# sloisel/MultiGridBarrier.jl

Measured on AMD Instinct MI355X. Metric: Newton iters/sec + wall-clock to converge, 2D P2 p-Laplace L=9, higher is better.
Workload: dtype f64

## Files before the change

### multigridbarrier.jl_amd/csrc/mf_launch_plan.hpp

```cpp
#pragma once
#include <algorithm>
#include <cstdint>
#include <cstdlib>
#include <vector>

#include "mf_analysis.hpp"

namespace mgbhip {

struct MfLaunch {
    int32_t first, count;
    int32_t cls;
    int32_t max_m, max_k;
    int32_t max_child = 0;
    bool tiny = false;
    bool wave = false;
    bool inv = false;
    bool iface = false;
    int32_t grec_first = -1;
};

constexpr int BIG_INV_MAX_M = 7000;
constexpr int GATHER_MAX_CHILD = 8;
constexpr int BIG_DIAG0_MIN_COUNT = 24;

struct MfSwitches {
    bool no_geo;
    bool old_big;
    bool merge_groups;
    bool packed_leaves;
    bool wave_small;
    int64_t inv_min_n;
    int64_t wave_min_n;
    bool gather_lds_maps;
    int gather_ct;
    static MfSwitches from_env() {
        auto on = [](const char* name) { const char* e = getenv(name); return e && e[0] == '1'; };
        auto num = [](const char* name, long long dflt) { const char* e = getenv(name); return e ? atoll(e) : dflt; };
        return {on("MGBHIP_NO_GEO"), on("MGBHIP_OLD_BIG"), !on("MGBHIP_NO_MERGE_GROUPS"), !on("MGBHIP_NO_PACKED_LEAVES"),
                !on("MGBHIP_NO_WAVE_SMALL"), num("MGBHIP_INV_MIN_N", 1024), num("MGBHIP_WAVE_MIN_N", 0),
                on("MGBHIP_GATHER_LDS_MAPS"), (int)num("MGBHIP_GATHER_CT", 0)};
    }
};

using LevelLaunches = std::vector<std::vector<MfLaunch>>;

inline MfLaunch launch_of_range(const MfPlan& plan, MfLaunch L, int32_t first, int32_t count) {
    L.first = first; L.count = count;
    L.max_m = 0; L.max_k = 0; L.max_child = 0;
    for (int32_t t = first; t < first + count; ++t) {
        L.max_m = std::max(L.max_m, plan.fronts[t].m);
        L.max_k = std::max(L.max_k, plan.fronts[t].k);
        L.max_child = std::max(L.max_child, plan.fronts[t].nchild);
    }
    return L;
}

inline void merge_straggler_groups(const MfPlan& plan, std::vector<MfLaunch>& G) {
    auto absorb = [&](size_t into, size_t from) {
        MfLaunch& A = G[into];
        const MfLaunch& B = G[from];
        A.first = B.first;
        A.count += B.count;
        A.max_k = std::max(A.max_k, B.max_k);
        A.max_child = std::max(A.max_child, B.max_child);
        G.erase(G.begin() + (long)from);
    };
    if (G.size() >= 2 && G.back().cls == 0 && G.back().inv) {
        int64_t lds_count = 0;
        bool ok = true;
        for (size_t g = 0; g + 1 < G.size(); ++g) { lds_count += G[g].count; ok = ok && !G[g].tiny && plan.fronts[G[g].first].m > 32; }
        if (ok && lds_count <= G.back().count)
            while (G.size() >= 2) absorb(G.size() - 1, G.size() - 2);
    }
    for (size_t g = 0; g + 1 < G.size();) {
        const bool next_lds = G[g + 1].cls != 0;
        if (next_lds && !G[g].tiny && (G[g].count < 256 || 4 * (int64_t)G[g].count < G[g + 1].count)) absorb(g + 1, g);
        else ++g;
    }
}

inline void split_interface_front(const MfPlan& plan, LevelLaunches& levels, bool inv_allowed) {
    const int32_t q = plan.iface_front;
    for (auto& G : levels) {
        for (size_t g = 0; g < G.size(); ++g) {
            const MfLaunch L = G[g];
            if (q < L.first || q >= L.first + L.count) continue;
            std::vector<MfLaunch> out;
            if (q > L.first) out.push_back(launch_of_range(plan, L, L.first, q - L.first));
            MfLaunch I = launch_of_range(plan, L, q, 1);
            I.cls = 0; I.tiny = false; I.wave = false; I.iface = true;
            I.inv = (I.max_m <= BIG_INV_MAX_M && inv_allowed);
            out.push_back(I);
            if (q + 1 < L.first + L.count) out.push_back(launch_of_range(plan, L, q + 1, L.first + L.count - q - 1));
// ... 57 lines not shown
        MfLaunch S{};
        for (auto& L : levels[l]) {
            if (!L.cls || L.tiny) { solves[l].push_back(L); continue; }
            if (S.count == 0) S = L;
            else {
                S.count += L.count;
                S.max_m = std::max(S.max_m, L.max_m);
                S.max_k = std::max(S.max_k, L.max_k);
            }
        }
        if (S.count) solves[l].insert(solves[l].begin(), S);
    }
    return solves;
}

inline std::vector<char> fronts_on_big_path(const MfPlan& plan, const LevelLaunches& levels) {
    std::vector<char> on_big_path(plan.fronts.size(), 0);
    for (auto& lev : levels)
        for (auto& L : lev)
            if (!L.cls)
                for (int32_t q = L.first; q < L.first + L.count; ++q) on_big_path[q] = 1;
    return on_big_path;
}

inline bool leaf_fronts_packable(const MfPlan& plan, const LevelLaunches& levels, const std::vector<char>& on_big_path) {
    bool any = false;
    for (auto& lev : levels)
        for (auto& L : lev)
            if (L.tiny)
                for (int32_t q = L.first; q < L.first + L.count; ++q) {
                    const int32_t par = plan.fronts[q].parent;
                    if (par >= 0 && on_big_path[par]) return false;
                    any = true;
                }
    return any;
}

enum MfAssembly : int32_t { MF_ASM_NONE = 0, MF_ASM_GATHER = 1, MF_ASM_COLS = 2 };
enum MfBlock0 : int32_t { MF_B0_NA = 0, MF_B0_GATHER = 1, MF_B0_DIAG0 = 2, MF_B0_STEP0 = 3 };
enum MfBackward : int32_t { MF_BWD_NA = 0, MF_BWD_K8 = 1, MF_BWD_K16 = 2, MF_BWD_GENERAL = 3 };

inline size_t big_gather_lds(const MfLaunch& L) { return (size_t)L.max_child * (size_t)L.max_m * sizeof(int32_t); }
inline MfAssembly big_assembly_kind(const MfLaunch& L) {
    if (L.cls) return MF_ASM_NONE;
    if (L.max_child < 1 || L.max_child > GATHER_MAX_CHILD || big_gather_lds(L) > 40 * 1024) return MF_ASM_COLS;
    return MF_ASM_GATHER;
}
inline MfBlock0 big_block0_kind(const MfLaunch& L, bool inv) {
    if (L.cls || !inv) return MF_B0_NA;
    if (!L.iface && big_assembly_kind(L) == MF_ASM_GATHER) return MF_B0_GATHER;
    return (L.iface || L.count >= BIG_DIAG0_MIN_COUNT) ? MF_B0_DIAG0 : MF_B0_STEP0;
}
inline int backward_small_kmax(const MfLaunch& L) { return L.max_k <= 8 ? 8 : (L.max_k <= 16 ? 16 : 0); }

constexpr int GATHER_MIN_WGS = 768;
inline int big_gather_ct(const MfLaunch& L, int forced) {
    if (forced == 8 || forced == 16 || forced == 32) return forced;
    int ct = 8;
    while (ct < 32 && (int64_t)L.count * ((L.max_m + 2 * ct - 1) / (2 * ct)) >= GATHER_MIN_WGS) ct *= 2;
    return ct;
}

struct GatherRec {
    int64_t map_off;
    int64_t base[GATHER_MAX_CHILD];
    int32_t ld[GATHER_MAX_CHILD];
    int32_t bs[GATHER_MAX_CHILD];
};

inline void build_gather_maps(const MfPlan& plan, LevelLaunches& levels, std::vector<GatherRec>& recs, std::vector<int32_t>& gmap) {
    recs.clear();
    gmap.clear();
    for (auto& lev : levels)
        for (auto& L : lev) {
            L.grec_first = -1;
            if (L.count == 0 || big_assembly_kind(L) != MF_ASM_GATHER) continue;
            L.grec_first = (int32_t)recs.size();
            for (int32_t q = L.first; q < L.first + L.count; ++q) {
                const Front& f = plan.fronts[q];
                GatherRec R{};
                R.map_off = (int64_t)gmap.size();
                gmap.resize(gmap.size() + (size_t)f.nchild * (size_t)f.m, -1);
                for (int32_t c = 0; c < f.nchild; ++c) {
                    const Front& ch = plan.fronts[plan.children[f.child_off + c]];
                    R.base[c] = ch.F_off + (int64_t)ch.k * ch.m + ch.k;
                    R.ld[c] = ch.m;
                    R.bs[c] = ch.m - ch.k;
                    int32_t* mp = gmap.data() + R.map_off + (int64_t)c * f.m;
                    for (int32_t j = 0; j < ch.m - ch.k; ++j) mp[plan.rel[ch.rel_off + j]] = j;
                }
                recs.push_back(R);
            }
        }
}

constexpr int MF_LAUNCH_ROW = 16;
inline int64_t launch_rows(const LevelLaunches& levels, const LevelLaunches& solves, bool leaf_packed, bool robust,
                           int32_t* out, int64_t cap) {
    int64_t n = 0;
    for (size_t l = 0; l < levels.size(); ++l) {
        int32_t bwd = 0;
        for (auto& S : solves[l])
            if (S.cls && !S.tiny) { const int km = backward_small_kmax(S); bwd = km == 8 ? MF_BWD_K8 : (km == 16 ? MF_BWD_K16 : MF_BWD_GENERAL); }
        for (auto& L : levels[l]) {
            if (n < cap && out) {
                const bool inv = L.inv && !robust;
                int32_t* r = out + n * MF_LAUNCH_ROW;
                r[0] = (int32_t)l; r[1] = L.first; r[2] = L.count; r[3] = L.cls; r[4] = L.max_m; r[5] = L.max_k; r[6] = L.max_child;
                r[7] = L.tiny; r[8] = L.wave; r[9] = inv; r[10] = L.iface; r[11] = L.tiny && leaf_packed;
                r[12] = big_assembly_kind(L); r[13] = big_block0_kind(L, inv); r[14] = (L.cls && !L.tiny) ? bwd : (int32_t)MF_BWD_NA; r[15] = 0;
            }
            ++n;
        }
    }
    return n;
}

}
```

### multigridbarrier.jl_amd/csrc/mf_numeric.hip

```cpp
#include <hip/hip_runtime.h>

#include <cstdio>

#include <algorithm>
#include <cstdlib>

#include "../../include/mgbhip.h"
#include "mf_solver.hpp"
#include "mf_device.hpp"
#include "mf_small.hpp"
#include "mf_big_subst.hpp"
#include "mf_big_inv.hpp"

namespace mgbhip {

namespace {

int32_t query_lds_cap() {
    if (hipFuncSetAttribute((const void*)mf_factor_small<8, true>, hipFuncAttributeMaxDynamicSharedMemorySize,
                            (int)factor_small_lds(128)) == hipSuccess)
        return 128;
    (void)hipGetLastError();
    return 88;
}
bool query_inv_optin() {
    if (hipFuncSetAttribute((const void*)mf_fwd_inv, hipFuncAttributeMaxDynamicSharedMemorySize, (int)fwd_inv_lds(BIG_INV_MAX_M)) == hipSuccess &&
        hipFuncSetAttribute((const void*)mf_bwd_inv, hipFuncAttributeMaxDynamicSharedMemorySize,
                            (int)bwd_inv_lds(BIG_INV_MAX_M, BIG_INV_MAX_M)) == hipSuccess)
        return true;
    (void)hipGetLastError();
    return false;
}

void build_gather_lists(const MfPlan& plan, const std::vector<char>& on_big_path, std::vector<FrontDev>& fd,
                        std::vector<int64_t>& ug_ptr, std::vector<int64_t>& ug_src) {
    for (int32_t i = 0; i < (int32_t)plan.fronts.size(); ++i) {
        const Front& f = plan.fronts[i];
        if (!on_big_path[i]) continue;
        fd[i].ug_off = (int64_t)ug_ptr.size();
        std::vector<int32_t> cnt((size_t)f.m + 1, 0);
        for (int32_t c = 0; c < f.nchild; ++c) {
            const Front& ch = plan.fronts[plan.children[f.child_off + c]];
            for (int32_t j = 0; j < ch.m - ch.k; ++j) cnt[plan.rel[ch.rel_off + j] + 1]++;
        }
        const int64_t base = (int64_t)ug_src.size();
        std::vector<int64_t> pos((size_t)f.m + 1);
        pos[0] = base;
        for (int32_t j = 0; j < f.m; ++j) pos[j + 1] = pos[j] + cnt[j + 1];
        ug_ptr.insert(ug_ptr.end(), pos.begin(), pos.end());
        ug_src.resize((size_t)pos[f.m]);
        std::vector<int64_t> fill(pos.begin(), pos.end() - 1);
        for (int32_t c = 0; c < f.nchild; ++c) {
            const Front& ch = plan.fronts[plan.children[f.child_off + c]];
            for (int32_t j = 0; j < ch.m - ch.k; ++j) ug_src[(size_t)fill[plan.rel[ch.rel_off + j]]++] = ch.u_off + j;
        }
    }
    if (ug_ptr.empty()) ug_ptr.push_back(0);
    if (ug_src.empty()) ug_src.push_back(0);
}

bool pack_leaf_fronts(const MfPlan& plan, const LevelLaunches& levels, const std::vector<char>& on_big_path,
                      std::vector<FrontDev>& fd) {
    if (!leaf_fronts_packable(plan, levels, on_big_path)) return false;
    for (auto& lev : levels)
        for (auto& L : lev)
            if (L.tiny)
                for (int32_t q = L.first; q < L.first + L.count; ++q) fd[q].packed = 1;
    return true;
}

std::vector<int32_t> remap_a_dst(const MfPlan& plan, const LevelLaunches& levels) {
    std::vector<int32_t> ad(plan.a_dst);
// ... 60 lines not shown
        const double one = 1.0;
        d_one.upload(&one, 1, st);
        MGB_HIP_CHECK(hipStreamSynchronize(st));
    }
    d_tbig.alloc(plan.front_idx.size() ? plan.front_idx.size() : 1);
    d_tsol.alloc(plan.front_idx.size() ? plan.front_idx.size() : 1);
    d_dvec.alloc(plan.front_idx.size() ? plan.front_idx.size() : 1);
    d_status.alloc(2);
    d_status.zero(st);
}

void MfSolver::analyze(int64_t n, const int32_t* rowptr, const int32_t* colidx, hipStream_t st,
                       const double* coords, int dim, bool protect_peeled, const int32_t* top, int64_t ntop) {
    const MfSwitches sw = MfSwitches::from_env();
    MfOptions opt;
    opt.protect_peeled = protect_peeled;
    opt.top = top;
    opt.ntop = ntop;
    opt.border = true;
    mf_analyze(n, rowptr, colidx, opt, plan, sw.no_geo ? nullptr : coords, dim);
    const int32_t nf = (int32_t)plan.fronts.size();
    std::vector<FrontDev> fd(nf);
    for (int32_t i = 0; i < nf; ++i) {
        const Front& f = plan.fronts[i];
        fd[i] = FrontDev{f.k, f.m, f.nchild, f.a_cnt, f.F_off, f.idx_off, f.u_off, f.child_off, f.rel_off, f.a_off, f.acol_off, -1, 0, 0};
    }
    upload_plan(st);

    lds_cap = query_lds_cap();
    const bool inv_ok = !sw.old_big && query_inv_optin();
    level_launches = classify_launches(plan, lds_cap, inv_ok, sw);
    level_solves = merge_level_solves(level_launches);
    uses_inv = false;
    const std::vector<char> on_big_path = fronts_on_big_path(plan, level_launches);
    int32_t max_big = 1;
    for (auto& lev : level_launches)
        for (auto& L : lev) {
            uses_inv = uses_inv || L.inv;
            if (!L.cls) max_big = std::max(max_big, L.count);
        }
    d_dscr.alloc((size_t)max_big * 2 * NB * NB);

    std::vector<int64_t> ug_ptr, ug_src;
    build_gather_lists(plan, on_big_path, fd, ug_ptr, ug_src);
    leaf_packed = sw.packed_leaves && pack_leaf_fronts(plan, level_launches, on_big_path, fd);
    d_ug_ptr.upload(ug_ptr, st);
    d_ug_src.upload(ug_src, st);
    std::vector<GatherRec> grec;
    std::vector<int32_t> gmap;
    if (!sw.gather_lds_maps) build_gather_maps(plan, level_launches, grec, gmap);
    gather_ct = sw.gather_ct;
    if (grec.empty()) { d_grec.release(); d_gmap.release(); }
    else { d_grec.upload(grec, st); d_gmap.upload(gmap, st); }
    d_fronts.upload(fd, st);
    h_fronts = fd;
    h_a_dst = remap_a_dst(plan, level_launches);
    d_a_dst.upload(h_a_dst, st);
    if (const char* e = getenv("MGBHIP_DEBUG"); e && atoi(e) >= 2) dump_plan(plan, level_launches);
    analyzed = true;
    MGB_HIP_CHECK(hipStreamSynchronize(st));
}

void MfSolver::set_direct_map(const int32_t* value_map, int64_t nnz, int64_t tail_base, hipStream_t st) {
    std::vector<int32_t> as(plan.a_src.size());
    for (size_t t = 0; t < as.size(); ++t) {
        const int64_t src = plan.a_src[t];
        const int64_t v = src < nnz ? (int64_t)value_map[src] : tail_base + (src - nnz);
        MGB_REQUIRE(v < (int64_t)INT32_MAX, "direct value index exceeds 32 bits");
        as[t] = (int32_t)v;
    }
    d_a_src_direct.upload(as, st);
    MGB_HIP_CHECK(hipStreamSynchronize(st));
}

void MfSolver::factor(const double* d_values, hipStream_t st, StageTimers* timers, bool direct, bool condensed) {
    MGB_REQUIRE(!direct || d_a_src_direct.n > 0, "MfSolver::factor: no direct value map");
    MGB_REQUIRE(!condensed || (direct && condensed_ok), "MfSolver::factor: condensed leaves are not enabled");
    MGB_REQUIRE(analyzed, "MfSolver::factor before analyze");
    const FactorArgs a{condensed ? d_fronts_c.p : d_fronts.p, d_children.p, d_rel.p,
                       condensed ? d_a_src_c.p : (direct ? d_a_src_direct.p : d_a_src.p), condensed ? d_a_dst_c.p : d_a_dst.p,
                       condensed ? d_a_colptr_c.p : d_a_colptr.p, d_values, d_arena.p, d_dscr.p, d_dvec.p, d_status.p, st,
                       d_grec.n ? d_grec.p : nullptr, d_gmap.p, gather_ct};
    if (timers) timers->begin("factor");
    factored_inv = !robust;
    if (!status_zero) MGB_HIP_CHECK(hipMemsetAsync(d_status.p, 0, sizeof(int32_t), st));
    status_zero = false;
    factored_condensed = condensed;
    int lvno = -1;
    for (auto& lev : level_launches) {
        LevelScope lvscope(timers, "fac", ++lvno);
        for (auto& L : lev) {
            if (L.count == 0) continue;
            if (condensed && lvno == 0) continue;
            if (L.tiny) launch_factor_tiny(a, L);
            else if (L.wave && L.cls <= 32) launch_factor_wave<32>(a, L);
            else if (L.wave) launch_factor_wave<48>(a, L);
            else if (L.cls) launch_factor_small(a, L);
            else {
                const bool inv = L.inv && !robust;
                const MfBlock0 b0 = big_block0_kind(L, inv);
                MGB_REQUIRE(!L.iface || (bool)iface_reduce, "MfSolver: interface front without a reduction hook");
                launch_big_assemble(a, L, b0 == MF_B0_GATHER);
                if (L.iface) {
                    const Front& fi = plan.fronts[L.first];
                    const int64_t tri = (int64_t)fi.m * (fi.m + 1) / 2;
                    d_ifpack.ensure((size_t)tri);
                    launch_tri_pack(fi.m, d_arena.p + fi.F_off, d_ifpack.p, false, st);
                    iface_reduce(d_ifpack.p, tri);
                    launch_tri_pack(fi.m, d_arena.p + fi.F_off, d_ifpack.p, true, st);
                }
                if (inv) {
                    if (b0 == MF_B0_DIAG0) launch_big_diag0(a, L, L.count);
                    launch_inv_steps(a, L, L.count, b0 == MF_B0_STEP0);
                } else
                    launch_subst_steps(a, L, L.count);
            }
        }
    }
    MGB_HIP_CHECK(hipGetLastError());
    if (timers) timers->end();
}

void MfSolver::solve(const double* d_b, double* d_x, hipStream_t st, StageTimers* timers) {
    MGB_REQUIRE(analyzed, "MfSolver::solve before analyze");
    if (timers) timers->begin("trisolve");
    const size_t n = (size_t)plan.n;
    MGB_HIP_CHECK(hipMemcpyAsync(d_bx.p, d_b, n * sizeof(double), hipMemcpyDeviceToDevice, st));
    MGB_HIP_CHECK(hipMemsetAsync(d_bx.p + n, 0, sizeof(double), st));
    forward_pass(d_bx.p, st, timers);
    backward_pass(d_xx.p, st, timers);
    MGB_HIP_CHECK(hipMemcpyAsync(d_x, d_xx.p, n * sizeof(double), hipMemcpyDeviceToDevice, st));
    MGB_HIP_CHECK(hipGetLastError());
    if (timers) timers->end();
}

// ... 175 lines not shown
```

### multigridbarrier.jl_amd/csrc/mf_small.hpp

```cpp
#pragma once
#include "mf_device.hpp"

namespace mgbhip {
namespace {

template <int NBT, bool PACKED>
__global__ void mf_factor_small(const FrontDev* __restrict__ fr, int32_t first,
                                const int32_t* __restrict__ children, const int32_t* __restrict__ rel,
                                const int32_t* __restrict__ a_src, const int32_t* __restrict__ a_dst,
                                const double* __restrict__ Hval, double* __restrict__ arena,
                                int32_t* __restrict__ status) {
    extern __shared__ double W[];
    const FrontDev F = fr[first + blockIdx.x];
    double* Fg = arena + F.F_off;
    const int m = F.m, k = F.k;
    const int tid = threadIdx.x, nt = blockDim.x;
    const int tx = tid % TX, ty = tid / TX, TYn = nt / TX;
    const int mm = PACKED ? m * (m + 1) / 2 : m * m;
    auto co = [m](int c) { return PACKED ? c * (m - 1) - c * (c - 1) / 2 : c * m; };
    double* S = W + mm;

    SP(0);
    int a_d0 = -1;
    double a_v0 = 0.0;
    if (tid < F.a_cnt) {
        a_d0 = a_dst[F.a_off + tid];
        a_v0 = Hval[a_src[F.a_off + tid]];
    }
    int64_t pU = 0, pR = 0;
    int32_t pM = 0, pB = 0;
    if (tid < min(CHILD_CHUNK, F.nchild)) {
        const FrontDev C = fr[children[F.child_off + tid]];
        child_update_desc(C, pU, pM);
        pR = C.rel_off;
        pB = C.m - C.k;
    }
    for (int i = tid; i < mm; i += nt) W[i] = 0.0;
    __syncthreads();
    if (a_d0 >= 0) W[a_d0] = a_v0;
    for (int t = tid + nt; t < F.a_cnt; t += nt) W[a_dst[F.a_off + t]] = Hval[a_src[F.a_off + t]];
    __syncthreads();
    SP(1);
    __shared__ int64_t cU[CHILD_CHUNK];
    __shared__ int64_t cR[CHILD_CHUNK];
    __shared__ int32_t cM[CHILD_CHUNK], cB[CHILD_CHUNK];
    __shared__ int32_t crl[128];
    __shared__ double prinv[32];
    for (int cbase = 0; cbase < F.nchild; cbase += CHILD_CHUNK) {
        const int nc = min(CHILD_CHUNK, F.nchild - cbase);
        __syncthreads();
        if (tid < nc) {
            if (cbase == 0) {
                cU[tid] = pU; cR[tid] = pR; cM[tid] = pM; cB[tid] = pB;
            } else {
                const FrontDev C = fr[children[F.child_off + cbase + tid]];
                int64_t u_; int32_t m_;
                child_update_desc(C, u_, m_);
                cU[tid] = u_;
                cR[tid] = C.rel_off;
                cM[tid] = m_;
                cB[tid] = C.m - C.k;
            }
        }
        __syncthreads();
        for (int c0 = 0; c0 < nc; c0 += 4) {
            if (nt == 256 && (c0 & 15) == 0) {
                const int ng = min(16, nc - c0);
                bool small16 = true;
                for (int u = 0; u < ng; ++u) small16 = small16 && cB[c0 + u] * cB[c0 + u] <= 64;
                if (small16) {
                    const int w = tid >> 6, e = tid & 63;
                    int dst[4];
                    double val[4];
#pragma unroll
                    for (int u = 0; u < 4; ++u) {
                        dst[u] = -1;
                        val[u] = 0.0;
                        const int c = c0 + 4 * w + u;
                        if (4 * w + u < ng) {
                            const int b = cB[c];
                            if (e < b * b) {
                                const int j = e / b, r = e - j * b;
                                if (r >= j) {
                                    const int32_t* rl = rel + cR[c];
                                    dst[u] = rl[r] + co(rl[j]);
                                    val[u] = arena[child_entry(cU[c], cM[c], j, r)];
                                }
                            }
                        }
                    }
#pragma unroll
                    for (int ph = 0; ph < 4; ++ph) {
                        if (4 * ph < ng) {
                            if (ph == w) {
#pragma unroll
                                for (int u = 0; u < 4; ++u) {
                                    if (dst[u] >= 0) W[dst[u]] += val[u];
                                    wave_sync();
                                }
                            }
                            __syncthreads();
                        }
                    }
                    c0 += 12;
                    continue;
                }
// ... 87 lines not shown
#pragma unroll
                for (int c = 0; c < NBT; ++c) {
                    S[c * m + r] = (c < nb) ? a[c] : 0.0;
                    if (c < nb) W[r + co(j0 + c)] = a[c] * prinv[c];
                }
            }
        }
        SPL(3);
        __syncthreads();
        SPL(4);
        {
            const int c0 = j0 + nb;
            const int T = (m - c0 + 15) >> 4;
            const int lane = tid & 63, fr16 = lane & 15, fk = lane >> 4;
            for (int tile = tid >> 6; tile < T * (T + 1) / 2; tile += nt >> 6) {
                int I = (int)((sqrtf(8.0f * (float)tile + 1.0f) - 1.0f) * 0.5f);
                while ((I + 1) * (I + 2) / 2 <= tile) ++I;
                while (I * (I + 1) / 2 > tile) --I;
                const int J = tile - I * (I + 1) / 2;
                const int r0 = c0 + 16 * I, cc0 = c0 + 16 * J;
                const int rr = min(r0 + fr16, m - 1), cc = min(cc0 + fr16, m - 1);
                double4_t acc = {0.0, 0.0, 0.0, 0.0};
#pragma unroll
                for (int kk = 0; kk < NBT / 4; ++kk) {
                    const int q = 4 * kk + fk;
                    const double sa = S[q * m + cc];
                    const double lb = (q < nb) ? W[rr + co(j0 + q)] : 0.0;
                    acc = __builtin_amdgcn_mfma_f64_16x16x4f64(sa, lb, acc, 0, 0, 0);
                }
#pragma unroll
                for (int i = 0; i < 4; ++i) {
                    const int col = cc0 + fk + 4 * i, row = r0 + fr16;
                    if (row < m && col < m && row >= col) W[row + co(col)] -= acc[i];
                }
            }
        }
        SPL(5);
        __syncthreads();
        SPL(6);
    }
    SP(3);
    if (bad && tid == 0) atomicOr(status, 1);
    if (PACKED) {
        for (int c = ty; c < m; c += TYn) {
            const int cc = co(c);
            for (int r = c + tx; r < m; r += TX) Fg[r + (int64_t)c * m] = W[cc + r];
        }
    } else {
        for (int i = tid; i < mm; i += nt) Fg[i] = W[i];
    }
    SP(4);
}

template <int MW>
__global__ __launch_bounds__(256) void mf_factor_wave(const FrontDev* __restrict__ fr, int32_t first, int32_t count,
                                                      const int32_t* __restrict__ children, const int32_t* __restrict__ rel,
                                                      const int32_t* __restrict__ a_src, const int32_t* __restrict__ a_dst,
                                                      const double* __restrict__ Hval, double* __restrict__ arena,
                                                      int32_t* __restrict__ status) {
    constexpr int PK = MW * (MW + 1) / 2;
    extern __shared__ double sh[];
#ifdef MGB_STEP_PROBE
#define WP(i) do { if (threadIdx.x == 0 && gridDim.x == 2048 && blockIdx.x == 1500) g_probe[8 + (i)] = wall_clock64(); } while (0)
#else
#define WP(i) do { } while (0)
#endif
    WP(0);
    const int lane = threadIdx.x & 63, wave = threadIdx.x >> 6;
    const int fi = blockIdx.x * 4 + wave;
    if (fi >= count) return;
    const FrontDev F = fr[first + fi];
    const int m = F.m, k = F.k;
    double* W = sh + (size_t)wave * PK;
    constexpr int WCH = 32;
    int64_t* cU = reinterpret_cast<int64_t*>(sh + (size_t)4 * PK) + wave * 2 * WCH;
    int64_t* cR = cU + WCH;
    int32_t* cM = reinterpret_cast<int32_t*>(reinterpret_cast<int64_t*>(sh + (size_t)4 * PK) + 4 * 2 * WCH) + wave * 2 * WCH;
    int32_t* cB = cM + WCH;
    auto pidx = [](int r, int c) { return c * MW - c * (c - 1) / 2 + (r - c); };
    int a_d0 = -1;
    double a_v0 = 0.0;
    if (lane < F.a_cnt) {
        a_d0 = a_dst[F.a_off + lane];
        a_v0 = Hval[a_src[F.a_off + lane]];
    }
    int64_t pU = 0, pR = 0;
    int32_t pM = 0, pB = 0;
    if (lane < min(WCH, F.nchild)) {
        const FrontDev C = fr[children[F.child_off + lane]];
        child_update_desc(C, pU, pM);
        pR = C.rel_off;
        pB = C.m - C.k;
    }
    for (int i = lane; i < PK; i += 64) W[i] = 0.0;
    wave_sync();
    WP(1);
    if (a_d0 >= 0) W[a_d0] = a_v0;
    for (int t = lane + 64; t < F.a_cnt; t += 64) W[a_dst[F.a_off + t]] = Hval[a_src[F.a_off + t]];
    wave_sync();
    WP(2);
    for (int cbase = 0; cbase < F.nchild; cbase += WCH) {
        const int nc = min(WCH, F.nchild - cbase);
        if (lane < nc) {
            if (cbase == 0) {
                cU[lane] = pU; cR[lane] = pR; cM[lane] = pM; cB[lane] = pB;
            } else {
                const FrontDev C = fr[children[F.child_off + cbase + lane]];
                int64_t u_; int32_t m_;
                child_update_desc(C, u_, m_);
                cU[lane] = u_;
                cR[lane] = C.rel_off;
                cM[lane] = m_;
                cB[lane] = C.m - C.k;
            }
        }
        wave_sync();
        for (int c0 = 0; c0 < nc; c0 += 16) {
            const int ng = min(16, nc - c0);
            bool small16 = true;
            for (int u = 0; u < ng; ++u) small16 = small16 && cB[c0 + u] * cB[c0 + u] <= 64;
            if (small16) {
                int dst[16];
                double val[16];
#pragma unroll
                for (int u = 0; u < 16; ++u) {
                    dst[u] = -1;
                    val[u] = 0.0;
                    if (u < ng) {
                        const int c = c0 + u, b = cB[c];
                        if (lane < b * b) {
                            const int j = (int)(((float)lane + 0.5f) * __builtin_amdgcn_rcpf((float)b)), r = lane - j * b;
                            if (r >= j) {
                                const int32_t* rl = rel + cR[c];
                                dst[u] = pidx(rl[r], rl[j]);
                                val[u] = arena[child_entry(cU[c], cM[c], j, r)];
                            }
                        }
                    }
                }
#pragma unroll
                for (int u = 0; u < 16; ++u) {
                    if (u < ng) {
                        if (dst[u] >= 0) W[dst[u]] += val[u];
                        wave_sync();
                    }
                }
            } else {
                for (int u = 0; u < ng; ++u) {
                    const int c = c0 + u, b = cB[c], mc = cM[c];
                    const int32_t* rl = rel + cR[c];
                    for (int e = lane; e < b * b; e += 256) {
                        int dd[4];
                        double vv[4];
#pragma unroll
                        for (int q = 0; q < 4; ++q) {
                            const int ee = e + 64 * q;
                            dd[q] = -1;
                            vv[q] = 0.0;
                            if (ee < b * b) {
                                const int j = ee / b, r = ee - j * b;
                                if (r >= j) {
                                    dd[q] = pidx(rl[r], rl[j]);
                                    vv[q] = arena[child_entry(cU[c], mc, j, r)];
                                }
                            }
                        }
#pragma unroll
                        for (int q = 0; q < 4; ++q)
                            if (dd[q] >= 0) W[dd[q]] += vv[q];
                    }
                    wave_sync();
                }
// ... 61 lines not shown
                dst[u] = -1;
                val[u] = 0.0;
                if (lane < bb[u]) {
                    dst[u] = rel[rr[u] + lane];
                    val[u] = uvec[ru[u] + lane];
                }
            }
#pragma unroll
            for (int u = 0; u < 4; ++u) {
                if (c0 + u >= nc) break;
                if (dst[u] >= 0) t[dst[u]] += val[u];
                for (int j = lane + 64; j < bb[u]; j += 64) t[rel[rr[u] + j]] += uvec[ru[u] + j];
                wave_sync();
            }
        }
    }
    const int r1 = lane + 64;
    double t0 = (lane < m) ? t[lane] : 0.0;
    double t1 = (r1 < m) ? t[r1] : 0.0;
#pragma unroll 4
    for (int j = 0; j < k; ++j) {
        const double* Lj = Fm + (int64_t)j * m;
        const double l0 = (lane > j && lane < m) ? Lj[lane] : 0.0;
        const double l1 = (r1 > j && r1 < m) ? Lj[r1] : 0.0;
        const double tj = (j < 64) ? readlane_f64(t0, j) : readlane_f64(t1, j - 64);
        t0 -= l0 * tj;
        t1 -= l1 * tj;
    }
    if (lane < m) {
        if (lane < k) y[idx[lane]] = t0 / Fm[lane + (int64_t)lane * m];
        else uvec[F.u_off + lane - k] = t0;
    }
    if (r1 < m) {
        if (r1 < k) y[idx[r1]] = t1 / Fm[r1 + (int64_t)r1 * m];
        else uvec[F.u_off + r1 - k] = t1;
    }
}

template <int KMAX>
__global__ __launch_bounds__(256) void mf_backward_small(const FrontDev* __restrict__ fr, int32_t first,
                                                         int32_t count,
                                                         const int32_t* __restrict__ front_idx,
                                                         const double* __restrict__ arena,
                                                         const double* __restrict__ y, double* __restrict__ x) {
    const int lane = threadIdx.x & 63, wave = threadIdx.x >> 6;
    const int fi = blockIdx.x * 4 + wave;
    if (fi >= count) return;
    const FrontDev F = fr[first + fi];
    const int m = F.m, k = F.k;
    const int32_t* idx = front_idx + F.idx_off;
    const double* Fm = arena + F.F_off;
    const int r1 = lane + 64;
    double t0 = 0.0, t1 = 0.0;
    if constexpr (KMAX > 0) {
        double l0[KMAX], l1[KMAX];
        const bool two = m > 64;
#pragma unroll
        for (int j = 0; j < KMAX; ++j) {
            l0[j] = (j < k && lane > j && lane < m) ? Fm[(int64_t)j * m + lane] : 0.0;
            l1[j] = (two && j < k && r1 < m) ? Fm[(int64_t)j * m + r1] : 0.0;
        }
        if (lane < m) t0 = (lane < k) ? y[idx[lane]] : x[idx[lane]];
        if (r1 < m) t1 = (r1 < k) ? y[idx[r1]] : x[idx[r1]];
#pragma unroll
        for (int j = KMAX - 1; j >= 0; --j) {
            if (j < k) {
                double s = l0[j] * t0;
                if (two) s += l1[j] * t1;
                s = wave_sum_f64(s);
                if (lane == j) t0 -= s;
            }
        }
    } else {
        if (lane < m) t0 = (lane < k) ? y[idx[lane]] : x[idx[lane]];
        if (r1 < m) t1 = (r1 < k) ? y[idx[r1]] : x[idx[r1]];
#pragma unroll 2
        for (int j = k - 1; j >= 0; --j) {
            const double* Lj = Fm + (int64_t)j * m;
            double s = 0.0;
            if (lane > j && lane < m) s += Lj[lane] * t0;
            if (r1 > j && r1 < m) s += Lj[r1] * t1;
            s = wave_sum_f64(s);
            if (lane == j) t0 -= s;
            if (r1 == j) t1 -= s;
        }
    }
    if (lane < k) x[idx[lane]] = t0;
    if (r1 < k) x[idx[r1]] = t1;
}

__global__ __launch_bounds__(256) void mf_factor_tiny(const FrontDev* __restrict__ fr, int32_t first, int32_t count,
                                                      const int32_t* __restrict__ a_src,
                                                      const int32_t* __restrict__ a_dst,
                                                      const double* __restrict__ Hval, double* __restrict__ arena,
                                                      int32_t* __restrict__ status) {
    __shared__ double Wt[16][136];
    __shared__ double colb[16][16];
    const int g = threadIdx.x >> 4, r = threadIdx.x & 15;
    const int fi = blockIdx.x * 16 + g;
    const bool on = fi < count;
    const FrontDev F = fr[first + (on ? fi : 0)];
    const int m = F.m, k = on ? F.k : 0;
    double* W = Wt[g];
    for (int i = r; i < 136; i += 16) W[i] = 0.0;
    wave_sync();
    if (on)
        for (int t = r; t < F.a_cnt; t += 16) W[a_dst[F.a_off + t]] = Hval[a_src[F.a_off + t]];
// ... 48 lines not shown
    double t = (row && r < k) ? b[myidx] : 0.0;
    double l[16];
#pragma unroll
    for (int j = 0; j < 16; ++j) l[j] = (row && j < k && r > j) ? Fm[tiny_entry(F, r, j)] : 0.0;
    const double dr = (row && r < k) ? Fm[tiny_entry(F, r, r)] : 1.0;
    int kmax = k;
    kmax = max(kmax, __shfl_xor(kmax, 16, 64));
    kmax = max(kmax, __shfl_xor(kmax, 32, 64));
#pragma unroll
    for (int j = 0; j < 16; ++j) {
        if (j >= kmax) break;
        const double tj = __shfl(t, j, 16);
        t -= l[j] * tj;
    }
    if (row) {
        if (r < k) y[myidx] = t / dr;
        else uvec[F.u_off + r - k] = t;
    }
}

__global__ __launch_bounds__(256) void mf_backward_tiny(const FrontDev* __restrict__ fr, int32_t first, int32_t count,
                                                        const int32_t* __restrict__ front_idx,
                                                        const double* __restrict__ arena,
                                                        const double* __restrict__ y, double* __restrict__ x) {
    const int g = threadIdx.x >> 4, r = threadIdx.x & 15;
    const int fi = blockIdx.x * 16 + g;
    const bool on = fi < count;
    const FrontDev F = fr[first + (on ? fi : 0)];
    const int m = F.m, k = on ? F.k : 0;
    const int32_t* idx = front_idx + F.idx_off;
    const double* Fm = arena + F.F_off;
    const bool row = on && r < m;
    const int myidx = row ? idx[r] : 0;
    double t = row ? ((r < k) ? y[myidx] : x[myidx]) : 0.0;
    double l[16];
#pragma unroll
    for (int j = 0; j < 16; ++j) l[j] = (row && j < k && r > j) ? Fm[tiny_entry(F, r, j)] : 0.0;
    int kmax = k;
    kmax = max(kmax, __shfl_xor(kmax, 16, 64));
    kmax = max(kmax, __shfl_xor(kmax, 32, 64));
#pragma unroll
    for (int j = 15; j >= 0; --j) {
        if (j >= kmax) continue;
        double s = l[j] * t;
        s = row16_sum_f64(s);
        if (r == j && j < k) t -= s;
    }
    if (row && r < k) x[myidx] = t;
}

inline size_t factor_small_lds(int cls) {
    return (size_t)((cls >= 88 ? cls * (cls + 1) / 2 : cls * cls) + 8 * cls) * sizeof(double);
}
inline void launch_factor_small(const FactorArgs& a, const MfLaunch& L) {
    const int threads = L.cls <= 16 ? 64 : (L.cls <= 32 ? 128 : 256);
    if (L.cls >= 88)
        hipLaunchKernelGGL((mf_factor_small<8, true>), dim3(L.count), dim3(threads), factor_small_lds(L.cls), a.st, a.fr, L.first,
                           a.children, a.rel, a.a_src, a.a_dst, a.values, a.arena, a.status);
    else
        hipLaunchKernelGGL((mf_factor_small<8, false>), dim3(L.count), dim3(threads), factor_small_lds(L.cls), a.st, a.fr, L.first,
                           a.children, a.rel, a.a_src, a.a_dst, a.values, a.arena, a.status);
}

template <int MW>
inline size_t factor_wave_lds() {
    return (size_t)4 * (MW * (MW + 1) / 2) * sizeof(double) + 4 * 64 * (sizeof(int64_t) + sizeof(int32_t));
}
template <int MW>
inline void launch_factor_wave(const FactorArgs& a, const MfLaunch& L) {
    hipLaunchKernelGGL(mf_factor_wave<MW>, dim3((L.count + 3) / 4), dim3(256), factor_wave_lds<MW>(), a.st, a.fr, L.first, L.count,
                       a.children, a.rel, a.a_src, a.a_dst, a.values, a.arena, a.status);
}

inline void launch_factor_tiny(const FactorArgs& a, const MfLaunch& L) {
    hipLaunchKernelGGL(mf_factor_tiny, dim3((L.count + 15) / 16), dim3(256), 0, a.st, a.fr, L.first, L.count, a.a_src, a.a_dst,
                       a.values, a.arena, a.status);
}

inline void launch_forward_tiny(const SolveArgs& a, const MfLaunch& L) {
    hipLaunchKernelGGL(mf_forward_tiny, dim3((L.count + 15) / 16), dim3(256), 0, a.st, a.fr, L.first, L.count, a.front_idx,
                       a.arena, a.b, a.y, a.uvec);
}
inline void launch_backward_tiny(const SolveArgs& a, const MfLaunch& L) {
    hipLaunchKernelGGL(mf_backward_tiny, dim3((L.count + 15) / 16), dim3(256), 0, a.st, a.fr, L.first, L.count, a.front_idx,
                       a.arena, a.y, a.x);
}

inline size_t forward_small_lds(int ts) { return (size_t)4 * ts * sizeof(double); }
inline void launch_forward_small(const SolveArgs& a, const MfLaunch& L) {
    const int ts = (L.max_m + 1) & ~1;
    hipLaunchKernelGGL(mf_forward_small, dim3((L.count + 3) / 4), dim3(256), forward_small_lds(ts), a.st, a.fr, L.first, L.count,
                       ts, a.front_idx, a.children, a.rel, a.arena, a.b, a.y, a.uvec);
}
template <int KMAX>
inline void launch_backward_small_k(const SolveArgs& a, const MfLaunch& L) {
    hipLaunchKernelGGL(mf_backward_small<KMAX>, dim3((L.count + 3) / 4), dim3(256), 0, a.st, a.fr, L.first, L.count, a.front_idx,
                       a.arena, a.y, a.x);
}
inline void launch_backward_small(const SolveArgs& a, const MfLaunch& L) {
    const int kmax = backward_small_kmax(L);
    if (kmax == 8) launch_backward_small_k<8>(a, L);
    else if (kmax == 16) launch_backward_small_k<16>(a, L);
    else launch_backward_small_k<0>(a, L);
}

}
}
```

### multigridbarrier.jl_amd/csrc/mf_solver.hpp

```cpp
#pragma once
#include <functional>

#include "common.hpp"
#include "mf_analysis.hpp"
#include "mf_launch_plan.hpp"
#include "kernels.hpp"

namespace mgbhip {

struct FrontDev {
    int32_t k, m, nchild, a_cnt;
    int64_t F_off, idx_off, u_off, child_off, rel_off, a_off, acol_off;
    int64_t ug_off;
    int32_t packed;
    int32_t pad_;
};

struct FactorArgs {
    const FrontDev* fr;
    const int32_t *children, *rel, *a_src, *a_dst, *a_colptr;
    const double* values;
    double *arena, *dscr, *dvec;
    int32_t* status;
    hipStream_t st;
    const GatherRec* grec;
    const int32_t* gmap;
    int gather_ct;
};
struct SolveArgs {
    const FrontDev* fr;
    const int32_t *front_idx, *children, *rel;
    const int64_t *ug_ptr, *ug_src;
    const double *arena, *dvec;
    const double* b;
    double *y, *x, *uvec, *tbig, *tsol;
    hipStream_t st;
};

class MfSolver {
   public:
    MfPlan plan;
    void analyze(int64_t n, const int32_t* rowptr, const int32_t* colidx, hipStream_t st,
                 const double* coords = nullptr, int dim = 0, bool protect_peeled = false,
                 const int32_t* top = nullptr, int64_t ntop = 0);
    std::function<void(double*, int64_t)> iface_reduce;
    void factor(const double* d_values, hipStream_t st, StageTimers* timers, bool direct = false, bool condensed = false);
    bool enable_condensed(int64_t N, int P, const int32_t* ucol, int64_t slack0, int64_t nnz, int64_t tail_base, hipStream_t st);
    bool condensed_ready() const { return condensed_ok; }
    bool leaves_packed() const { return leaf_packed; }
    const LeafDesc* leaf_desc() const { return d_leaf_desc.p; }
    double* arena() { return d_arena.p; }
    int32_t* leaf_status() { return d_status.p + 1; }
    const int32_t* status_flags() const { return d_status.p; }
    int32_t* status_flags_rw() { return d_status.p; }
    void flags_cleared() { status_zero = true; leaf_zero = true; }
    bool leaf_flag_zero() const { return leaf_zero; }
    void leaf_flag_used() { leaf_zero = false; }
    void set_direct_map(const int32_t* value_map, int64_t nnz, int64_t tail_base, hipStream_t st);
    bool has_direct_map() const { return d_a_src_direct.n > 0; }
    void solve(const double* d_b, double* d_x, hipStream_t st, StageTimers* timers);
    void solve_border(double* d_x_np1, hipStream_t st, StageTimers* timers);
    void chain_stats(double* out8) const;
    int64_t launches(int32_t* out, int64_t cap) const;
    int status(hipStream_t st);
    void status_async(int32_t* h_dst, hipStream_t st) const;
    static int status_from(const int32_t* flags2, bool with_leaves) {
        return (flags2[0] || (with_leaves && flags2[1])) ? MGBHIP_ERR_NOT_SPD : MGBHIP_OK;
    }
    bool factored_condensed = false;
    bool analyzed = false;
    bool robust = false;
    bool has_inverse_path() const { return uses_inv; }
    bool factored_inv = false;

   private:
    void upload_plan(hipStream_t st);
    SolveArgs solve_args(const double* d_b, double* d_x, hipStream_t st) const {
        return {d_fronts.p, d_front_idx.p, d_children.p, d_rel.p, d_ug_ptr.p, d_ug_src.p, d_arena.p, d_dvec.p, d_b, d_y.p, d_x,
                d_uvec.p, d_tbig.p, d_tsol.p, st};
    }
    void forward_pass(const double* d_b_np1, hipStream_t st, StageTimers* timers);
    void backward_pass(double* d_x_np1, hipStream_t st, StageTimers* timers);
    DevBuf<double> d_bx, d_xx, d_one;
    DevBuf<FrontDev> d_fronts;
    DevBuf<int32_t> d_front_idx, d_children, d_rel, d_a_src, d_a_src_direct, d_a_dst, d_a_colptr;
    DevBuf<GatherRec> d_grec;
    DevBuf<int32_t> d_gmap;
    DevBuf<int64_t> d_ug_ptr, d_ug_src;
    DevBuf<double> d_arena, d_uvec, d_y, d_tbig, d_tsol, d_dscr, d_dvec;
    DevBuf<double> d_ifpack;
    DevBuf<int32_t> d_status;
    bool condensed_ok = false;
    bool leaf_packed = false;
    std::vector<FrontDev> h_fronts;
    std::vector<int32_t> h_a_dst;
    DevBuf<FrontDev> d_fronts_c;
    DevBuf<int32_t> d_a_src_c, d_a_dst_c, d_a_colptr_c;
    DevBuf<LeafDesc> d_leaf_desc;
    std::vector<std::vector<MfLaunch>> level_launches;
    std::vector<std::vector<MfLaunch>> level_solves;
    int gather_ct = 0;
    int32_t lds_cap = 88;
    bool uses_inv = false;
    bool y_border_one = false;
    bool y_zero = false;
    bool status_zero = false, leaf_zero = false;
};

}
```

Baseline: 680.7.

## Precompute child records and conflict-free wave scatter lists for multifrontal factor

Builds compact per-child records (update base, stride, rel offset, border size) on the host, so the small and wave factor kernels no longer load full FrontDev structs through the children indirection. For wave-class fronts it also precomputes packed extend-add scatter words grouped into rounds with no destination conflicts, so lanes can accumulate into LDS without atomics and with one barrier per round. It further adds a one-row KMAX=24 backward-substitution specialization. The cost is extra device buffers, more template instantiations and host preprocessing at analysis time. The round loop adds a barrier per round, which could be slower than the old per-child path on fronts with many rounds.

```diff
diff --git a/multigridbarrier.jl_amd/csrc/mf_launch_plan.hpp b/multigridbarrier.jl_amd/csrc/mf_launch_plan.hpp
--- a/multigridbarrier.jl_amd/csrc/mf_launch_plan.hpp
+++ b/multigridbarrier.jl_amd/csrc/mf_launch_plan.hpp
@@ -1,5 +1,6 @@
 #pragma once
 #include <algorithm>
+#include <climits>
 #include <cstdint>
 #include <cstdlib>
 #include <vector>
@@ -34,12 +35,13 @@
     int64_t wave_min_n;
     bool gather_lds_maps;
     int gather_ct;
+    bool child_lists;
     static MfSwitches from_env() {
         auto on = [](const char* name) { const char* e = getenv(name); return e && e[0] == '1'; };
         auto num = [](const char* name, long long dflt) { const char* e = getenv(name); return e ? atoll(e) : dflt; };
         return {on("MGBHIP_NO_GEO"), on("MGBHIP_OLD_BIG"), !on("MGBHIP_NO_MERGE_GROUPS"), !on("MGBHIP_NO_PACKED_LEAVES"),
                 !on("MGBHIP_NO_WAVE_SMALL"), num("MGBHIP_INV_MIN_N", 1024), num("MGBHIP_WAVE_MIN_N", 0),
-                on("MGBHIP_GATHER_LDS_MAPS"), (int)num("MGBHIP_GATHER_CT", 0)};
+                on("MGBHIP_GATHER_LDS_MAPS"), (int)num("MGBHIP_GATHER_CT", 0), !on("MGBHIP_NO_CHILD_LISTS")};
     }
 };
 
@@ -203,6 +205,7 @@
     return (L.iface || L.count >= BIG_DIAG0_MIN_COUNT) ? MF_B0_DIAG0 : MF_B0_STEP0;
 }
 inline int backward_small_kmax(const MfLaunch& L) { return L.max_k <= 8 ? 8 : (L.max_k <= 16 ? 16 : 0); }
+inline bool backward_small_one_row24(const MfLaunch& L) { return L.max_k > 16 && L.max_k <= 24 && L.max_m <= 64; }
 
 constexpr int GATHER_MIN_WGS = 768;
 inline int big_gather_ct(const MfLaunch& L, int forced) {
@@ -245,6 +248,99 @@
         }
 }
 
+struct ChildRec {
+    int64_t U;
+    int64_t rel_off;
+    int32_t M;
+    int32_t b;
+};
+
+inline void build_child_records(const MfPlan& plan, const std::vector<char>& packed, std::vector<ChildRec>& recs) {
+    recs.resize(plan.children.size());
+    for (size_t i = 0; i < plan.children.size(); ++i) {
+        const int32_t q = plan.children[i];
+        const Front& ch = plan.fronts[q];
+        ChildRec& R = recs[i];
+        if (packed[(size_t)q]) {
+            R.U = ch.F_off + (int64_t)ch.k * ch.m - (ch.k * (ch.k - 1)) / 2;
+            R.M = -(ch.m - ch.k);
+        } else {
+            R.U = ch.F_off + (int64_t)ch.k * ch.m + ch.k;
+            R.M = ch.m;
+        }
+        R.rel_off = ch.rel_off;
+        R.b = ch.m - ch.k;
+    }
+}
+
+inline int32_t packed_tri_index(int32_t stride, int32_t r, int32_t c) { return c * stride - c * (c - 1) / 2 + (r - c); }
+
+constexpr int WAVE_LIST_MAX_CHILD = 64;
+constexpr uint32_t WAVE_LIST_PAD = 0xffffffffu;
+constexpr uint32_t wave_list_word(int32_t dst, int32_t child, int32_t j, int32_t r, int32_t round) {
+    return (uint32_t)dst | ((uint32_t)j << 11) | ((uint32_t)r << 14) | ((uint32_t)child << 17) | ((uint32_t)round << 23);
+}
+constexpr int32_t wave_word_dst(uint32_t w) { return (int32_t)(w & 2047u); }
+constexpr int32_t wave_word_j(uint32_t w) { return (int32_t)((w >> 11) & 7u); }
+constexpr int32_t wave_word_r(uint32_t w) { return (int32_t)((w >> 14) & 7u); }
+constexpr int32_t wave_word_child(uint32_t w) { return (int32_t)((w >> 17) & 63u); }
+constexpr int32_t wave_word_round(uint32_t w) { return (int32_t)(w >> 23); }
+
+struct WaveListRec {
+    int32_t off;
+    uint16_t total, nrounds;
+};
+
+inline void build_wave_lists(const MfPlan& plan, const LevelLaunches& levels, std::vector<WaveListRec>& wl, std::vector<uint32_t>& words) {
+    wl.assign(plan.fronts.size(), WaveListRec{-1, 0, 0});
+    words.clear();
+    std::vector<int32_t> last(2048, -1);
+    std::vector<uint32_t> entries;
+    std::vector<int32_t> round_of, fill;
+    for (auto& lev : levels)
+        for (auto& L : lev) {
+            if (!L.wave) continue;
+            const int32_t stride = L.cls <= 32 ? 32 : 48;
+            for (int32_t q = L.first; q < L.first + L.count; ++q) {
+                const Front& f = plan.fronts[q];
+                if (f.nchild > WAVE_LIST_MAX_CHILD) continue;
+                bool fits = true;
+                entries.clear();
+                for (int32_t c = 0; c < f.nchild && fits; ++c) {
+                    const Front& ch = plan.fronts[plan.children[f.child_off + c]];
+                    const int32_t b = ch.m - ch.k;
+                    const int32_t* rel = plan.rel.data() + ch.rel_off;
+                    fits = b <= 8;
+                    for (int32_t j = 0; j < b && fits; ++j)
+                        for (int32_t r = j; r < b; ++r) {
+                            if (rel[j] < 0 || rel[r] < rel[j] || rel[r] >= stride) { fits = false; break; }
+                            entries.push_back(wave_list_word(packed_tri_index(stride, rel[r], rel[j]), c, j, r, 0));
+                        }
+                }
+                if (!fits || words.size() + entries.size() > (size_t)INT32_MAX) continue;
+                round_of.resize(entries.size());
+                fill.clear();
+                for (size_t e = 0; e < entries.size(); ++e) {
+                    int32_t& ld = last[(size_t)wave_word_dst(entries[e])];
+                    size_t rd = (size_t)(ld + 1);
+                    while (rd < fill.size() && fill[rd] == 64) ++rd;
+                    if (rd == fill.size()) fill.push_back(0);
+                    ++fill[rd];
+                    ld = round_of[e] = (int32_t)rd;
+                }
+                const size_t base = words.size();
+                words.resize(base + entries.size());
+                int32_t start = 0;
+                for (int32_t& n : fill) { const int32_t cnt = n; n = start; start += cnt; }
+                for (size_t e = 0; e < entries.size(); ++e) {
+                    words[base + (size_t)fill[(size_t)round_of[e]]++] = entries[e] | wave_list_word(0, 0, 0, 0, round_of[e]);
+                    last[(size_t)wave_word_dst(entries[e])] = -1;
+                }
+                wl[(size_t)q] = WaveListRec{(int32_t)base, (uint16_t)entries.size(), (uint16_t)fill.size()};
+            }
+        }
+}
+
 constexpr int MF_LAUNCH_ROW = 16;
 inline int64_t launch_rows(const LevelLaunches& levels, const LevelLaunches& solves, bool leaf_packed, bool robust,
                            int32_t* out, int64_t cap) {
diff --git a/multigridbarrier.jl_amd/csrc/mf_numeric.hip b/multigridbarrier.jl_amd/csrc/mf_numeric.hip
--- a/multigridbarrier.jl_amd/csrc/mf_numeric.hip
+++ b/multigridbarrier.jl_amd/csrc/mf_numeric.hip
@@ -3,6 +3,7 @@
 #include <cstdio>
 
 #include <algorithm>
+#include <chrono>
 #include <cstdlib>
 
 #include "../../include/mgbhip.h"
@@ -17,7 +18,9 @@
 namespace {
 
 int32_t query_lds_cap() {
-    if (hipFuncSetAttribute((const void*)mf_factor_small<8, true>, hipFuncAttributeMaxDynamicSharedMemorySize,
+    if (hipFuncSetAttribute((const void*)mf_factor_small<8, true, true>, hipFuncAttributeMaxDynamicSharedMemorySize,
+                            (int)factor_small_lds(128)) == hipSuccess &&
+        hipFuncSetAttribute((const void*)mf_factor_small<8, true, false>, hipFuncAttributeMaxDynamicSharedMemorySize,
                             (int)factor_small_lds(128)) == hipSuccess)
         return 128;
     (void)hipGetLastError();
@@ -184,6 +187,23 @@
     gather_ct = sw.gather_ct;
     if (grec.empty()) { d_grec.release(); d_gmap.release(); }
     else { d_grec.upload(grec, st); d_gmap.upload(gmap, st); }
+    std::vector<ChildRec> crec;
+    std::vector<WaveListRec> wlist;
+    std::vector<uint32_t> wwords;
+    child_lists = sw.child_lists;
+    if (child_lists) {
+        const auto t0 = std::chrono::steady_clock::now();
+        std::vector<char> packed((size_t)nf);
+        for (int32_t i = 0; i < nf; ++i) packed[(size_t)i] = (char)fd[i].packed;
+        build_child_records(plan, packed, crec);
+        build_wave_lists(plan, level_launches, wlist, wwords);
+        if (const char* e = getenv("MGBHIP_DEBUG"); e && atoi(e) >= 2)
+            fprintf(stderr, "[mgbhip] child records: %zu, wave lists: %zu words, built in %.1f ms\n", crec.size(), wwords.size(),
+                    1e3 * std::chrono::duration<double>(std::chrono::steady_clock::now() - t0).count());
+        if (crec.empty()) crec.push_back(ChildRec{});
+        if (wwords.empty()) wwords.push_back(WAVE_LIST_PAD);
+        d_crec.upload(crec, st); d_wlist.upload(wlist, st); d_wwords.upload(wwords, st);
+    } else { d_crec.release(); d_wlist.release(); d_wwords.release(); }
     d_fronts.upload(fd, st);
     h_fronts = fd;
     h_a_dst = remap_a_dst(plan, level_launches);
@@ -212,7 +232,8 @@
     const FactorArgs a{condensed ? d_fronts_c.p : d_fronts.p, d_children.p, d_rel.p,
                        condensed ? d_a_src_c.p : (direct ? d_a_src_direct.p : d_a_src.p), condensed ? d_a_dst_c.p : d_a_dst.p,
                        condensed ? d_a_colptr_c.p : d_a_colptr.p, d_values, d_arena.p, d_dscr.p, d_dvec.p, d_status.p, st,
-                       d_grec.n ? d_grec.p : nullptr, d_gmap.p, gather_ct};
+                       d_grec.n ? d_grec.p : nullptr, d_gmap.p, gather_ct,
+                       child_lists ? d_crec.p : nullptr, d_wlist.p, d_wwords.p};
     if (timers) timers->begin("factor");
     factored_inv = !robust;
     if (!status_zero) MGB_HIP_CHECK(hipMemsetAsync(d_status.p, 0, sizeof(int32_t), st));
diff --git a/multigridbarrier.jl_amd/csrc/mf_small.hpp b/multigridbarrier.jl_amd/csrc/mf_small.hpp
--- a/multigridbarrier.jl_amd/csrc/mf_small.hpp
+++ b/multigridbarrier.jl_amd/csrc/mf_small.hpp
@@ -4,9 +4,10 @@
 namespace mgbhip {
 namespace {
 
-template <int NBT, bool PACKED>
+template <int NBT, bool PACKED, bool REC>
 __global__ void mf_factor_small(const FrontDev* __restrict__ fr, int32_t first,
-                                const int32_t* __restrict__ children, const int32_t* __restrict__ rel,
+                                const int32_t* __restrict__ children, const ChildRec* __restrict__ crec,
+                                const int32_t* __restrict__ rel,
                                 const int32_t* __restrict__ a_src, const int32_t* __restrict__ a_dst,
                                 const double* __restrict__ Hval, double* __restrict__ arena,
                                 int32_t* __restrict__ status) {
@@ -30,10 +31,15 @@
     int64_t pU = 0, pR = 0;
     int32_t pM = 0, pB = 0;
     if (tid < min(CHILD_CHUNK, F.nchild)) {
-        const FrontDev C = fr[children[F.child_off + tid]];
-        child_update_desc(C, pU, pM);
-        pR = C.rel_off;
-        pB = C.m - C.k;
+        if constexpr (REC) {
+            const ChildRec R = crec[F.child_off + tid];
+            pU = R.U; pM = R.M; pR = R.rel_off; pB = R.b;
+        } else {
+            const FrontDev C = fr[children[F.child_off + tid]];
+            child_update_desc(C, pU, pM);
+            pR = C.rel_off;
+            pB = C.m - C.k;
+        }
     }
     for (int i = tid; i < mm; i += nt) W[i] = 0.0;
     __syncthreads();
@@ -52,6 +58,9 @@
         if (tid < nc) {
             if (cbase == 0) {
                 cU[tid] = pU; cR[tid] = pR; cM[tid] = pM; cB[tid] = pB;
+            } else if constexpr (REC) {
+                const ChildRec R = crec[F.child_off + cbase + tid];
+                cU[tid] = R.U; cR[tid] = R.rel_off; cM[tid] = R.M; cB[tid] = R.b;
             } else {
                 const FrontDev C = fr[children[F.child_off + cbase + tid]];
                 int64_t u_; int32_t m_;
@@ -245,9 +254,11 @@
     SP(4);
 }
 
-template <int MW>
+template <int MW, bool LISTS>
 __global__ __launch_bounds__(256) void mf_factor_wave(const FrontDev* __restrict__ fr, int32_t first, int32_t count,
-                                                      const int32_t* __restrict__ children, const int32_t* __restrict__ rel,
+                                                      const int32_t* __restrict__ children, const ChildRec* __restrict__ crec,
+                                                      const WaveListRec* __restrict__ wlist, const uint32_t* __restrict__ wwords,
+                                                      const int32_t* __restrict__ rel,
                                                       const int32_t* __restrict__ a_src, const int32_t* __restrict__ a_dst,
                                                       const double* __restrict__ Hval, double* __restrict__ arena,
                                                       int32_t* __restrict__ status) {
@@ -279,7 +290,33 @@
     }
     int64_t pU = 0, pR = 0;
     int32_t pM = 0, pB = 0;
-    if (lane < min(WCH, F.nchild)) {
+    constexpr int WLT = 8;
+    WaveListRec wl{-1, 0, 0};
+    int wl_off = -1, wl_total = 0, wl_rounds = 0;
+    uint32_t ww[WLT] = {};
+    auto list_words = [&](uint32_t (&w)[WLT], int e0) {
+#pragma unroll
+        for (int t = 0; t < WLT; ++t) {
+            const int e = e0 + 64 * t + lane;
+            w[t] = e < wl_total ? wwords[wl_off + e] : WAVE_LIST_PAD;
+        }
+    };
+    if constexpr (LISTS) {
+        wl = wlist[first + fi];
+        wl_off = __builtin_amdgcn_readfirstlane(wl.off);
+        wl_total = __builtin_amdgcn_readfirstlane((int)wl.total);
+        wl_rounds = __builtin_amdgcn_readfirstlane((int)wl.nrounds);
+        if (wl_off >= 0) {
+            if (lane < F.nchild) {
+                const ChildRec R = crec[F.child_off + lane];
+                pU = R.U; pM = R.M;
+            }
+            list_words(ww, 0);
+        } else if (lane < min(WCH, F.nchild)) {
+            const ChildRec R = crec[F.child_off + lane];
+            pU = R.U; pM = R.M; pR = R.rel_off; pB = R.b;
+        }
+    } else if (lane < min(WCH, F.nchild)) {
         const FrontDev C = fr[children[F.child_off + lane]];
         child_update_desc(C, pU, pM);
         pR = C.rel_off;
@@ -290,13 +327,49 @@
     WP(1);
     if (a_d0 >= 0) W[a_d0] = a_v0;
     for (int t = lane + 64; t < F.a_cnt; t += 64) W[a_dst[F.a_off + t]] = Hval[a_src[F.a_off + t]];
+    const bool listed = LISTS && wl_off >= 0;
+    if (listed && lane < F.nchild) {
+        static_assert(2 * WCH == WAVE_LIST_MAX_CHILD, "the records of a list front are staged by one lane each");
+        cU[lane] = pU;
+        cM[lane] = pM;
+    }
     wave_sync();
     WP(2);
-    for (int cbase = 0; cbase < F.nchild; cbase += WCH) {
+    if (listed) {
+        for (int e0 = 0; e0 < wl_total; e0 += 64 * WLT) {
+            double vv[WLT];
+#pragma unroll
+            for (int t = 0; t < WLT; ++t) {
+                vv[t] = 0.0;
+                if (ww[t] != WAVE_LIST_PAD) {
+                    const int c = wave_word_child(ww[t]);
+                    vv[t] = arena[child_entry(cU[c], cM[c], wave_word_j(ww[t]), wave_word_r(ww[t]))];
+                }
+            }
+            uint32_t wn[WLT];
+            list_words(wn, e0 + 64 * WLT);
+            const int q0 = wave_word_round((uint32_t)__builtin_amdgcn_readfirstlane((int)ww[0]));
+            for (int q = q0; q < wl_rounds; ++q) {
+                int d = -1;
+                double v = 0.0;
+#pragma unroll
+                for (int t = 0; t < WLT; ++t)
+                    if (wave_word_round(ww[t]) == q) { d = wave_word_dst(ww[t]); v = vv[t]; }
+                if (d >= 0) W[d] += v;
+                wave_sync();
+            }
+#pragma unroll
+            for (int t = 0; t < WLT; ++t) ww[t] = wn[t];
+        }
+    }
+    for (int cbase = 0; cbase < (listed ? 0 : F.nchild); cbase += WCH) {
         const int nc = min(WCH, F.nchild - cbase);
         if (lane < nc) {
             if (cbase == 0) {
                 cU[lane] = pU; cR[lane] = pR; cM[lane] = pM; cB[lane] = pB;
+            } else if constexpr (LISTS) {
+                const ChildRec R = crec[F.child_off + cbase + lane];
+                cU[lane] = R.U; cR[lane] = R.rel_off; cM[lane] = R.M; cB[lane] = R.b;
             } else {
                 const FrontDev C = fr[children[F.child_off + cbase + lane]];
                 int64_t u_; int32_t m_;
@@ -310,7 +383,7 @@
         wave_sync();
         for (int c0 = 0; c0 < nc; c0 += 16) {
             const int ng = min(16, nc - c0);
-            bool small16 = true;
+            bool small16 = !LISTS;
             for (int u = 0; u < ng; ++u) small16 = small16 && cB[c0 + u] * cB[c0 + u] <= 64;
             if (small16) {
                 int dst[16];
@@ -478,7 +551,21 @@
     const double* Fm = arena + F.F_off;
     const int r1 = lane + 64;
     double t0 = 0.0, t1 = 0.0;
-    if constexpr (KMAX > 0) {
+    if constexpr (KMAX == 24) {
+        double l0[KMAX];
+#pragma unroll
+        for (int j = 0; j < KMAX; ++j) l0[j] = (j < k && lane > j && lane < m) ? Fm[(int64_t)j * m + lane] : 0.0;
+        if (lane < m) t0 = (lane < k) ? y[idx[lane]] : x[idx[lane]];
+#pragma unroll
+        for (int j = KMAX - 1; j >= 0; --j) {
+            if (j < k) {
+                double s = 0.0;
+                if (lane > j && lane < m) s += l0[j] * t0;
+                s = wave_sum_f64(s);
+                if (lane == j) t0 -= s;
+            }
+        }
+    } else if constexpr (KMAX > 0) {
         double l0[KMAX], l1[KMAX];
         const bool two = m > 64;
 #pragma unroll
@@ -633,14 +720,15 @@
 inline size_t factor_small_lds(int cls) {
     return (size_t)((cls >= 88 ? cls * (cls + 1) / 2 : cls * cls) + 8 * cls) * sizeof(double);
 }
+template <bool PACKED, bool REC>
+inline void launch_factor_small_as(const FactorArgs& a, const MfLaunch& L) {
+    const int threads = L.cls <= 16 ? 64 : (L.cls <= 32 ? 128 : 256);
+    hipLaunchKernelGGL((mf_factor_small<8, PACKED, REC>), dim3(L.count), dim3(threads), factor_small_lds(L.cls), a.st, a.fr, L.first,
+                       a.children, a.crec, a.rel, a.a_src, a.a_dst, a.values, a.arena, a.status);
+}
 inline void launch_factor_small(const FactorArgs& a, const MfLaunch& L) {
-    const int threads = L.cls <= 16 ? 64 : (L.cls <= 32 ? 128 : 256);
-    if (L.cls >= 88)
-        hipLaunchKernelGGL((mf_factor_small<8, true>), dim3(L.count), dim3(threads), factor_small_lds(L.cls), a.st, a.fr, L.first,
-                           a.children, a.rel, a.a_src, a.a_dst, a.values, a.arena, a.status);
-    else
-        hipLaunchKernelGGL((mf_factor_small<8, false>), dim3(L.count), dim3(threads), factor_small_lds(L.cls), a.st, a.fr, L.first,
-                           a.children, a.rel, a.a_src, a.a_dst, a.values, a.arena, a.status);
+    if (L.cls >= 88) a.crec ? launch_factor_small_as<true, true>(a, L) : launch_factor_small_as<true, false>(a, L);
+    else a.crec ? launch_factor_small_as<false, true>(a, L) : launch_factor_small_as<false, false>(a, L);
 }
 
 template <int MW>
@@ -649,8 +737,12 @@
 }
 template <int MW>
 inline void launch_factor_wave(const FactorArgs& a, const MfLaunch& L) {
-    hipLaunchKernelGGL(mf_factor_wave<MW>, dim3((L.count + 3) / 4), dim3(256), factor_wave_lds<MW>(), a.st, a.fr, L.first, L.count,
-                       a.children, a.rel, a.a_src, a.a_dst, a.values, a.arena, a.status);
+    if (a.crec)
+        hipLaunchKernelGGL((mf_factor_wave<MW, true>), dim3((L.count + 3) / 4), dim3(256), factor_wave_lds<MW>(), a.st, a.fr, L.first,
+                           L.count, a.children, a.crec, a.wlist, a.wwords, a.rel, a.a_src, a.a_dst, a.values, a.arena, a.status);
+    else
+        hipLaunchKernelGGL((mf_factor_wave<MW, false>), dim3((L.count + 3) / 4), dim3(256), factor_wave_lds<MW>(), a.st, a.fr, L.first,
+                           L.count, a.children, a.crec, a.wlist, a.wwords, a.rel, a.a_src, a.a_dst, a.values, a.arena, a.status);
 }
 
 inline void launch_factor_tiny(const FactorArgs& a, const MfLaunch& L) {
@@ -682,6 +774,7 @@
     const int kmax = backward_small_kmax(L);
     if (kmax == 8) launch_backward_small_k<8>(a, L);
     else if (kmax == 16) launch_backward_small_k<16>(a, L);
+    else if (a.one_row24 && backward_small_one_row24(L)) launch_backward_small_k<24>(a, L);
     else launch_backward_small_k<0>(a, L);
 }
 
diff --git a/multigridbarrier.jl_amd/csrc/mf_solver.hpp b/multigridbarrier.jl_amd/csrc/mf_solver.hpp
--- a/multigridbarrier.jl_amd/csrc/mf_solver.hpp
+++ b/multigridbarrier.jl_amd/csrc/mf_solver.hpp
@@ -26,6 +26,9 @@
     const GatherRec* grec;
     const int32_t* gmap;
     int gather_ct;
+    const ChildRec* crec;
+    const WaveListRec* wlist;
+    const uint32_t* wwords;
 };
 struct SolveArgs {
     const FrontDev* fr;
@@ -35,6 +38,7 @@
     const double* b;
     double *y, *x, *uvec, *tbig, *tsol;
     hipStream_t st;
+    bool one_row24;
 };
 
 class MfSolver {
@@ -77,7 +81,7 @@
     void upload_plan(hipStream_t st);
     SolveArgs solve_args(const double* d_b, double* d_x, hipStream_t st) const {
         return {d_fronts.p, d_front_idx.p, d_children.p, d_rel.p, d_ug_ptr.p, d_ug_src.p, d_arena.p, d_dvec.p, d_b, d_y.p, d_x,
-                d_uvec.p, d_tbig.p, d_tsol.p, st};
+                d_uvec.p, d_tbig.p, d_tsol.p, st, child_lists};
     }
     void forward_pass(const double* d_b_np1, hipStream_t st, StageTimers* timers);
     void backward_pass(double* d_x_np1, hipStream_t st, StageTimers* timers);
@@ -86,6 +90,9 @@
     DevBuf<int32_t> d_front_idx, d_children, d_rel, d_a_src, d_a_src_direct, d_a_dst, d_a_colptr;
     DevBuf<GatherRec> d_grec;
     DevBuf<int32_t> d_gmap;
+    DevBuf<ChildRec> d_crec;
+    DevBuf<WaveListRec> d_wlist;
+    DevBuf<uint32_t> d_wwords;
     DevBuf<int64_t> d_ug_ptr, d_ug_src;
     DevBuf<double> d_arena, d_uvec, d_y, d_tbig, d_tsol, d_dscr, d_dvec;
     DevBuf<double> d_ifpack;
@@ -100,6 +107,7 @@
     std::vector<std::vector<MfLaunch>> level_launches;
     std::vector<std::vector<MfLaunch>> level_solves;
     int gather_ct = 0;
+    bool child_lists = false;
     int32_t lds_cap = 88;
     bool uses_inv = false;
     bool y_border_one = false;
```

Measured after the change: 688.6, median of 3. About the same (+1.2%).
